# flyish/NoahGameFrame

Measured on AMD Instinct MI355X. Metric: entity-ticks/sec (update+dirty-diff+fanout) at 1M entities/GPU, 1/2/4/8 GPUs, higher is better.
Workload: dtype int64/f64; 1 GPU; BASELINE config[1]: 1048576 NPC/Player entities per GPU in one scene, 4096 groups x 256, 8 players/group, heartbeats HPRegen 1s/MPRegen 2s/Move 0.1s/Patrol 3s/Poison 0.5s, 100 ms frames; entities_per_gpu=1048576, groups=4096, players_per_group=8, parallelism=scene-shard x1

## Files before the change

### noahgameframe_amd/csrc/nfgpu_device.hpp

```cpp
#pragma once
#include <hip/hip_runtime.h>
#include <stdint.h>

#include "../../include/nfgpu.h"

namespace nfgpu {

constexpr int kTPB = 256;
constexpr int kTile = 256;
#ifndef NFGPU_RTILE
#define NFGPU_RTILE 64
#endif
constexpr int kRTile = NFGPU_RTILE;
static_assert(kRTile >= 1 && kRTile <= 64, "a record tile is at most one wave of slots");
constexpr uint32_t kRrcHost = 0x03FFFFFFu;
constexpr int kRrcSitShift = 26;

constexpr unsigned kErrMsgCap = 4, kErrTouch = 8, kErrFanBound = 16, kErrRemain = 32;

struct alignas(64) Ctrl {
    unsigned err, pad_u[3];
    unsigned long long n_ev, n_fi, n_re, n_msgs;
    unsigned long long msg_extent, n_msgs_ptiles;
    unsigned long long bytes_tick, bytes_rec, bytes_fan, pad2;
};

struct alignas(16) SchedHot {
    int64_t next;
    int32_t remain;
    uint32_t state;
};
constexpr uint32_t kStPresent = 1, kStForever = 2, kStFired = 4, kStStep = 8;
__host__ __device__ __forceinline__ int64_t st_step(uint32_t st) { return (int64_t)((int32_t)st >> 4); }
__host__ __device__ __forceinline__ uint32_t st_pack_step(int64_t step) {
    return (step >= -(1ll << 27) && step < (1ll << 27)) ? (kStStep | ((uint32_t)step << 4)) : 0u;
}
struct alignas(16) SchedCold {
    int64_t start;
    int32_t all;
    float interval;
};

constexpr unsigned kAblPrograms = 4;
constexpr unsigned kAblPerKind = 8;
constexpr unsigned kAblWaves6 = 16, kAblWaves8 = 32;
constexpr unsigned kAblWaves5 = 8192;
constexpr unsigned kAblNoRun = 512, kAblNoLoads = 1024, kAblNoEmit = 2048;
constexpr unsigned kAblNoWriteBack = 1u << 18, kAblNoSchedStore = 1u << 19;
constexpr unsigned kAblNoFiStore = 128, kAblNoEvStore = 256;
constexpr unsigned kAblGroupColumns = 1u << 20, kAblSigGroups = 1u << 21;
constexpr unsigned kAblNoPad = 1u << 22;
constexpr unsigned kAblFanWin16 = 1u << 24, kAblFanWin32 = 1u << 25;
constexpr unsigned kAblFan1 = 1u << 26;
constexpr unsigned kAblFanNoWin = 1u << 30;
constexpr unsigned kAblTinyTcap = 1u << 27;
constexpr unsigned kAblForceMsgCap = 1u << 29;
typedef uint32_t u32x4_a4 __attribute__((ext_vector_type(4), aligned(4)));
typedef uint32_t u32x2_a4 __attribute__((ext_vector_type(2), aligned(4)));
constexpr int64_t kColPad = 2304;
constexpr unsigned kAblScanInFrame = 131072;
constexpr unsigned kAblScanKernel = 1u << 28;
constexpr int kLbMaxTiles = 256;
constexpr unsigned kAblNoFuse = 4096;
constexpr unsigned kAblCheckRem = 64;
constexpr int32_t kRemUnset = (int32_t)0x80000001;

__host__ __device__ inline uint32_t rec_pos(uint64_t used, uint64_t rowm, int r) {
    const uint64_t below = (1ull << r) - 1;
    return ((used >> r) & 1) ? (uint32_t)__builtin_popcountll(used & below)
                             : (uint32_t)(__builtin_popcountll(used & rowm) + __builtin_popcountll(~used & rowm & below));
}
__host__ __device__ inline uint64_t rec_rowm(int rows) { return rows >= 64 ? ~0ull : ((1ull << rows) - 1); }

struct RecOp {
    int32_t kind, rec, col, code;
    int64_t a, b, c;
};

constexpr int kMaxU = 16, kMaxW = 12;
constexpr uint8_t kNoU = 0xFF;
constexpr int kCellPid = 0x10000;
constexpr uint32_t kNoCell = 0xFFFFFFFFu;
__host__ __device__ __forceinline__ uint32_t cell_rec(uint32_t c) { return (c >> 10) & 7u; }
__host__ __device__ __forceinline__ uint32_t cell_row(uint32_t c) { return (c >> 4) & 63u; }
__host__ __device__ __forceinline__ uint32_t cell_col(uint32_t c) { return c & 15u; }
// ... 110 lines not shown
    uint32_t ablate;
    RecOpX rops[NFK_MAX_REC_OPS];
    int32_t n_rops;
    uint32_t rop_kinds;
    unsigned long long* tally;
    int32_t n_w, n_u;
    int32_t u_pid[kMaxU];
    uint64_t* u_col[kMaxU];
    int32_t u_str[kMaxU];
    int32_t u_order[kMaxW];
    uint32_t u_lower[kMaxW];
    uint32_t u_cmask[NFK_MAX_CLASSES];
    int32_t n_tiles, n_rtiles;
    int32_t ev_tcap, fi_tcap, re_tcap;
    uint32_t* t_ev;
    uint32_t* t_fi;
    uint32_t* t_re;
    uint32_t* t_msg;
    uint32_t* ev_base;
    uint32_t* fi_base;
    uint32_t* re_base;
    uint32_t* msg_base;
    uint64_t* lb_st;
    uint32_t* lb_cnt;
    uint32_t lb_epoch;
    int32_t lb_rank;
    uint32_t msg_tcap;
    int32_t fuse_fan;
    int32_t fuse_rec;
    uint32_t msg_rb0, msg_rtcap;
    int32_t lds_words;
    int32_t xcd_map;
    uint32_t* ev_slot; uint32_t* ev_pid; uint64_t* ev_old; uint64_t* ev_new; uint32_t* ev_moff;
    uint32_t* fi_slot; uint32_t* fi_kind; int32_t* fi_remain;
    uint32_t* re_rrc; uint64_t* re_old; uint64_t* re_new; uint32_t* re_moff;
    uint32_t* msg_rcpt; int64_t msg_cap;
    uint64_t* ev_old_h; uint64_t* ev_new_h;
    unsigned* err_host;
};

constexpr int kErrHostWords = 16;
__device__ __forceinline__ void dev_error(const Dev& d, unsigned bit) {
    atomicOr(&d.ctrl->err, bit);
    if (d.err_host) __hip_atomic_store(d.err_host + __builtin_ctz(bit), 1u, __ATOMIC_RELAXED, __HIP_MEMORY_SCOPE_SYSTEM);
}

constexpr int kTallyN = 64, kTallyTick = 0, kTallyRec = 1, kTallyFan = 2;
// ... 120 lines not shown
```

### noahgameframe_amd/csrc/nfgpu_host.hip

```cpp
#include <algorithm>
#include <chrono>
#include <cmath>
#include <cstdlib>
#include <cstdio>
#include <cstring>
#include <functional>
#include <map>
#include <memory>
#include <numeric>
#include <string>
#include <unordered_map>
#include <vector>

#include <mutex>
#include <thread>

#include <rocprim/device/device_radix_sort.hpp>
#include <rocprim/device/device_scan.hpp>

#include "nfgpu_jit.hpp"
#include "nfgpu_kernels.hip"
#include "../../include/nfgpu_guidmap.hpp"
#include "nfgpu_pool.hpp"

// ... 959 lines not shown

std::mutex g_jit_mu;
std::map<std::string, std::pair<hipFunction_t, hipFunction_t>> g_jit;

void build_jit(World* w) {
    w->jit_fn = nullptr;
    w->jit_chain_fn = nullptr;
    const char* env = getenv("NFGPU_JIT");
    if (env && env[0] == '0') {
        w->jit_msg = "disabled (NFGPU_JIT=0)";
        return;
    }
    if (!w->u_ok) {
        w->jit_msg = "working set does not fit k_tick (k_tick_touch runs)";
        return;
    }
    const int u = std::max(w->d.n_u, 1);
    int waves = (w->d.ablate & (kAblWaves6 | kAblWaves8 | kAblWaves5)) ? tick_waves(w->d.n_u, w->d.ablate) : kWavesJit;
    if (const char* ew = getenv("NFGPU_JIT_WAVES")) waves = std::max(1, std::min(8, atoi(ew)));
    const char* es = getenv("NFGPU_JIT_SPEC");
    const bool spec = es && es[0] == '1';
    uint32_t nt = kJitNtDefault;
    if (const char* en = getenv("NFGPU_JIT_NT")) nt = (uint32_t)strtoul(en, nullptr, 0);
    bool lb = ((int64_t)std::max(w->d.N, 1) + kTile - 1) / kTile <= kLbMaxTiles;
    if (const char* el = getenv("NFGPU_JIT_LB")) lb = el[0] == '1';
    const std::string src = jit_schema_source(w->tab, w->d, spec, nt, lb);
    int dev = 0;
    (void)hipGetDevice(&dev);
    const std::string key = std::to_string(dev) + "|" + std::to_string(waves) + "|" + std::to_string(u) + "|" + src;
    std::lock_guard<std::mutex> lk(g_jit_mu);
    auto it = g_jit.find(key);
    if (it == g_jit.end()) {
        JitBuild b = jit_compile(src, waves, u);
        hipModule_t mod = nullptr;
        hipFunction_t fn = nullptr, cfn = nullptr;
        if (!b.ok || hipModuleLoadData(&mod, b.code.data()) != hipSuccess ||
            hipModuleGetFunction(&fn, mod, b.lowered.c_str()) != hipSuccess ||
            hipModuleGetFunction(&cfn, mod, b.lowered_chain.c_str()) != hipSuccess) {
            w->jit_msg = "hipRTC build failed: " + b.log.substr(0, 2000);
            return;
        }
        it = g_jit.emplace(key, std::make_pair(fn, cfn)).first;
    }
    w->jit_fn = it->second.first;
    w->jit_chain_fn = it->second.second;
    w->jit_lb = lb;
    w->jit_waves = waves;
// ... 988 lines not shown
    set_working_set(w);
    ALLOC(w->pl_slot_w, (size_t)cap * 4);
    ALLOC(w->slot_obj_d, (size_t)cap * 4);
    ALLOC(w->fan_desc_w, (size_t)cap * 8);
    d.fan_desc = w->fan_desc_w;
    {
        const char* ab = getenv("NFGPU_ABLATE");
        d.ablate = ab ? (uint32_t)strtoul(ab, nullptr, 0) : 0u;
    }
    d.pl_slot = w->pl_slot_w;
    d.ev_tcap = kTile * std::max(w->n_dst_union, 1);
    d.fi_tcap = kTile * std::max(NK, 1);
    d.re_tcap = (int32_t)(kRTile * std::max<size_t>(rec_events_per_ent, 1));
    const size_t nt = cap / kTile, nrt = cap / kRTile;
    const size_t ev_n = nt * d.ev_tcap, fi_n = nt * d.fi_tcap, re_n = d.has_recops ? nrt * d.re_tcap : 1;
    ALLOC(d.t_ev, nt * 4);
    ALLOC(d.t_fi, nt * 4);
    ALLOC(d.t_re, nrt * 4);
    ALLOC(d.t_msg, (nt + nrt) * 4);
    ALLOC(d.ev_base, (nt + 1) * 4);
    ALLOC(d.fi_base, (nt + 1) * 4);
    ALLOC(d.re_base, (nrt + 1) * 4);
    ALLOC(d.msg_base, (nt + nrt + 1) * 4);
    ALLOC(d.lb_st, std::min<size_t>(nt, kLbMaxTiles) * 4 * 8);
    ALLOC(d.lb_cnt, 64);
    d.msg_cap = w->cfg.msg_capacity > 0 ? w->cfg.msg_capacity : (int64_t)cap * 32;
    if (d.msg_cap > 0xFFFFFFFFll) return fail(NFK_ERR_ARG, "msg_capacity must fit 32-bit offsets");
    ALLOC(d.ev_slot, ev_n * 4);
    ALLOC(d.ev_pid, ev_n * 4);
    ALLOC(d.ev_old, ev_n * 8);
    ALLOC(d.ev_new, ev_n * 8);
    ALLOC(d.ev_moff, ev_n * 4);
    if (w->cfg.n_obj) {
        ALLOC(d.ev_old_h, ev_n * 8);
        ALLOC(d.ev_new_h, ev_n * 8);
    }
    ALLOC(d.fi_slot, fi_n * 4);
    ALLOC(d.fi_kind, fi_n * 4);
    ALLOC(d.fi_remain, fi_n * 4);
    ALLOC(d.re_rrc, re_n * 4);
    ALLOC(d.re_old, re_n * 8);
    ALLOC(d.re_new, re_n * 8);
    ALLOC(d.re_moff, re_n * 4);
    ALLOC(d.msg_rcpt, d.msg_cap * 4);
    d.tab = w->tab_d;
    d.ctrl = w->ctrl;
    d.n_rops = nro;
    d.rop_kinds = w->tab.kind_has_recop;
// ... 64 lines not shown
        std::vector<uint64_t> fd(cap, kDeadDesc);
        std::vector<int32_t> pls(cap, 0), so(cap, -1);
        for (size_t i = 0; i < meta.slot.size(); i++) {
            fd[meta.slot[i]] = meta.desc[i];
            pls[meta.slot[i]] = meta.pl[i];
            so[meta.slot[i]] = meta.obj[i];
        }
        HIPCHK(hipMemcpy(w->fan_desc_w, fd.data(), (size_t)cap * 8, hipMemcpyHostToDevice));
        HIPCHK(hipMemcpy(w->pl_slot_w, pls.data(), (size_t)cap * 4, hipMemcpyHostToDevice));
        HIPCHK(hipMemcpy(w->slot_obj_d, so.data(), (size_t)cap * 4, hipMemcpyHostToDevice));
    }
    HIPCHK(hipMemset(d.e_flags, 0, cap));
    HIPCHK(hipMemset(d.ext_head, 0, (size_t)cap * 4));
    HIPCHK(hipMemset(d.rs_head, 0, (size_t)cap * 4));
    HIPCHK(hipMemset(d.fired_mask, 0, (size_t)cap * 4));
    HIPCHK(hipMemset(d.t_ev, 0, nt * 4));
    HIPCHK(hipMemset(d.t_fi, 0, nt * 4));
    HIPCHK(hipMemset(d.t_re, 0, nrt * 4));
    HIPCHK(hipMemset(d.t_msg, 0, (nt + nrt) * 4));
    HIPCHK(hipMemset(d.ev_base, 0, (nt + 1) * 4));
    HIPCHK(hipMemset(d.fi_base, 0, (nt + 1) * 4));
    HIPCHK(hipMemset(d.re_base, 0, (nrt + 1) * 4));
    HIPCHK(hipMemset(d.msg_base, 0, (nt + nrt + 1) * 4));
    HIPCHK(hipMemset(d.lb_st, 0, std::min<size_t>(nt, kLbMaxTiles) * 4 * 8));
    HIPCHK(hipMemset(d.lb_cnt, 0, 64));
    w->lb_epoch = 0;
    for (auto& v : w->init_props) std::vector<uint64_t>().swap(v);
    for (auto& v : w->init_rcells) std::vector<uint64_t>().swap(v);
    build_jit(w);
    {
        const size_t room = (size_t)w->n_obj + (size_t)w->n_obj / 4 + 4096;
        w->gh.reserve(room);
        w->gd.reserve(room);
        w->guid.reserve(room);
        w->scene.reserve(room);
        w->group.reserve(room);
        w->cls.reserve(room);
        w->isplayer.reserve(room);
        w->slot_of_obj.reserve(room);
        w->alive.reserve(room);
        w->src_row.reserve(room);
        w->m_flag.reserve(room);
        if (!w->ins_rows) {
            const size_t c = 1024;
            HIPCHK(hipMalloc((void**)&w->ins_rows, c * (size_t)w->row_words * 8));
            w->ins_cap = c;
        }
    }
// ... 878 lines not shown
    return NFK_OK;
}

int nfk_import_objects(void* world, int32_t n, const int64_t* gh, const int64_t* gd, const int32_t* scene,
                       const int32_t* group, const uint8_t* cls, const uint8_t* isplayer, const uint64_t* rows_dev) {
    World* w = (World*)world;
    if (!w) return fail(NFK_ERR_ARG, "null world");
    return import_common(w, n, gh, gd, scene, group, cls, isplayer, rows_dev, hipMemcpyDeviceToDevice);
}

int nfk_spawn_objects(void* world, int32_t n, const int64_t* gh, const int64_t* gd, const int32_t* scene,
                      const int32_t* group, const uint8_t* cls, const uint8_t* isplayer, const uint64_t* props) {
    World* w = (World*)world;
    if (!w || (n > 0 && !props)) return fail(NFK_ERR_ARG, "null argument");
    if (!w->committed) return fail(NFK_ERR_STATE, "commit first (before it, use nfk_create_objects)");
    std::vector<uint64_t> rows((size_t)std::max(n, 0) * w->row_words, 0);
    for (int32_t i = 0; i < n; i++)
        memcpy(&rows[(size_t)i * w->row_words], props + (size_t)i * w->n_pw, (size_t)w->n_pw * 8);
    return import_common(w, n, gh, gd, scene, group, cls, isplayer, rows.data(), hipMemcpyHostToDevice);
}

static int execute_frame(World* w, int64_t now_ms, bool calls_only) {
    if (!w->committed) return fail(NFK_ERR_STATE, "commit first");
    if (const unsigned e = err_host_bits(w); e & (kErrFanBound | kErrTouch))
        return fail(NFK_ERR_DEVICE, std::string("device error of an earlier frame: ") +
                                        ((e & kErrFanBound) ? "a tile's fan-out exceeded its bound" : "touch list overflow") +
                                        " (nfk_summary_get reports and clears it)");
    using clk = std::chrono::steady_clock;
    const bool trace = getenv("NFGPU_TRACE_EXEC") != nullptr;
    clk::time_point tp[6];
    tp[0] = clk::now();
    {
        if (!w->mplan) w->mplan.reset(new MemPlan());
        MemPlan& mp = *w->mplan;
        int r = plan_membership(w, mp);
        if (r) return r;
        const int rf = check_fanout(w);
        r = commit_membership(w, mp);
        if (rf) return drop_window(w, rf);
        if (r) return drop_window(w, r);
    }
    if (const char* inj = getenv("NFGPU_INJECT_EXEC_FAIL"); inj && inj[0] == '1')
        return drop_window(w, fail(NFK_ERR_CAPACITY, "injected failure after the membership changes"));
    if (w->cfg.n_obj) w->xops_h.resize(w->xops.size(), 0);
    Dev d = w->d;
    d.now = now_ms;

    tp[1] = clk::now();
    const size_t n_xdev = w->xq_n, n_xq = n_xdev + w->xops.size(), n_hq = w->hops.size();
// ... 460 lines not shown
                                                       : w->last_rec_msgs + w->last_rec_msgs / 4) + 1024;
        if (tcap * d.n_tiles <= kMsgStrideLimit) {
            if (need > w->d.msg_cap) {
                HIPCHK(hipStreamSynchronize(w->stream));
                int r = regrow(w, (void**)&w->d.msg_rcpt, (size_t)need * 4);
                if (r) {
                    w->d.msg_cap = 0;
                    return drop_window(w, r);
                }
                w->d.msg_cap = need;
                d.msg_rcpt = w->d.msg_rcpt;
                d.msg_cap = need;
            }
            d.msg_tcap = (uint32_t)tcap;
            if (rfuse) {
                d.fuse_rec = 1;
                d.msg_rb0 = (uint32_t)(tcap * d.n_tiles);
                d.msg_rtcap = (uint32_t)rtcap;
            }
        }
    }
    d.fuse_fan = d.msg_tcap != 0;
    const bool cells = d.n_u > 0 && d.u_pid[d.n_u - 1] >= kCellPid;
    d.lb_rank = (d.fuse_fan && !d.has_recops && d.n_tiles && d.n_tiles <= kLbMaxTiles &&
                 !(d.ablate & kAblScanKernel) && (!(use_u && w->jit_fn) || w->jit_lb)) ? 1 : 0;
    if (d.lb_rank) {
        if (++w->lb_epoch == 0xFFFFFFFFu) {
            HIPCHK(hipMemsetAsync(w->d.lb_st, 0, std::min<size_t>(w->obj_of_slot.size() / kTile, kLbMaxTiles) * 4 * 8,
                                  w->stream));
            w->lb_epoch = 1;
        }
        d.lb_epoch = w->lb_epoch;
    }
    w->last_tcap = d.msg_tcap;
    w->last_rtcap = d.fuse_rec ? d.msg_rtcap : 0u;
    if (!calls_only) w->chain_ran = false;
    if (!calls_only && (w->chain_watch[0] | w->chain_watch[1]) && d.N) {
        uint32_t kinds = 0;
        int64_t wops = 0;
        for (int k = 0; k < d.n_kind; k++)
            for (int i = 0; i < w->tab.nops[k]; i++) {
                const nfk_op& op = w->tab.ops[k][i];
                const bool prop_op = op.code == NFK_OP_IADD_CLAMP || op.code == NFK_OP_FLERP ||
                                     op.code == NFK_OP_FAFFINE || op.code == NFK_OP_ISET || op.code == NFK_OP_FSET;
                if (prop_op && op.dst < 128 && ((w->chain_watch[op.dst >> 6] >> (op.dst & 63)) & 1)) {
                    kinds |= 1u << k;
                    wops++;
                }
            }
        static const bool no_closure = getenv("NFGPU_CHAIN_NO_CLOSURE") && getenv("NFGPU_CHAIN_NO_CLOSURE")[0] == '1';
        if (kinds && !no_closure) {
            auto bit = [](uint64_t (&m)[2], uint32_t p) {
// ... 78 lines not shown
                else hipLaunchKernelGGL((k_chain_u<16, DynSchema>), dim3((unsigned)nt), dim3(kTPB), 0, w->stream, d, cd, cc, tcap, kinds, w0, w1);
            } else {
                hipLaunchKernelGGL(k_chain, dim3((unsigned)nt), dim3(kTPB), 0, w->stream, d, w->chain_d, w->chain_cnt_d, tcap,
                                   kinds, w->chain_watch[0], w->chain_watch[1]);
            }
            HIPCHK(hipGetLastError());
            w->chain_ran = true;
            w->chain_tiles = nt;
        }
    }
    if (d.n_tiles) {
        TimeScope ts(w, KT_TICK);
        size_t lds = (size_t)std::max(d.n_w, 1) * kTPB * 8 + (size_t)std::max(d.n_kind, 1) * kTPB * 4;
        const bool jit = use_u && w->jit_fn;
        if (d.fuse_fan) {
            const int waves = jit ? w->jit_waves : tick_waves(d.n_u, d.ablate);
            lds = std::max(lds, (size_t)(163840 / waves - 2560) & ~(size_t)1023);
        }
        d.lds_words = (int32_t)(lds / 4);
        {
            static const int xm = getenv("NFGPU_TICK_XCD") ? atoi(getenv("NFGPU_TICK_XCD")) : 1;
            d.xcd_map = xm;
        }
        const dim3 g((unsigned)d.n_tiles), b(kTPB);
        if (jit) {
            void* args[] = {&d};
            HIPCHK(hipModuleLaunchKernel(w->jit_fn, (unsigned)d.n_tiles, 1, 1, kTPB, 1, 1, (unsigned)lds, w->stream,
                                         args, nullptr));
        } else if (use_u && cells) {
            if (d.n_u <= 8 && !(d.ablate & kAblWaves6))
                hipLaunchKernelGGL((k_tick<kWavesU8, 8, DynSchemaCells>), g, b, lds, w->stream, d);
            else if (d.n_u <= 12 && !(d.ablate & kAblWaves6))
                hipLaunchKernelGGL((k_tick<kWavesU12, 12, DynSchemaCells>), g, b, lds, w->stream, d);
            else
                hipLaunchKernelGGL((k_tick<6, 16, DynSchemaCells>), g, b, lds, w->stream, d);
        } else if (use_u && d.n_u <= 8 && !(d.ablate & kAblWaves6))
            hipLaunchKernelGGL((k_tick<kWavesU8, 8>), g, b, lds, w->stream, d);
        else if (use_u && d.n_u <= 12 && !(d.ablate & kAblWaves6))
            hipLaunchKernelGGL((k_tick<kWavesU12, 12>), g, b, lds, w->stream, d);
        else if (use_u)
            hipLaunchKernelGGL((k_tick<6, 16>), g, b, lds, w->stream, d);
        else
            hipLaunchKernelGGL(k_tick_touch, dim3((unsigned)d.n_tiles), dim3(kTPB), 0, w->stream, d);
        HIPCHK(hipGetLastError());
    }
    if (d.has_recops && d.n_rtiles) {
        TimeScope ts(w, KT_REC);
        constexpr int kWpb = kTPB / 64;
        const dim3 g((unsigned)((d.n_rtiles + kWpb - 1) / kWpb)), b(kTPB);
        if (nrss)
// ... 196 lines not shown
    }
    out->n_prop_events = (int64_t)c.n_ev;
    out->n_rec_events = (int64_t)c.n_re;
    out->n_fired = (int64_t)c.n_fi;
    out->n_msgs = frame_msgs(w, c);
    {
        out->alg_bytes_tick = (int64_t)(tb[0] - w->last_bytes[0]);
        out->alg_bytes_rec = (int64_t)(tb[1] - w->last_bytes[1]);
        out->alg_bytes_fan = (int64_t)(tb[2] - w->last_bytes[2]);
        for (int k = 0; k < 3; k++) w->last_bytes[k] = tb[k];
    }
    if ((c.err & kErrMsgCap) && !(c.err & ~kErrMsgCap)) {
        int r = regrow_fanout(w, c);
        if (r) return r;
    }
    w->last_rec_msgs = frame_msgs(w, c) - (int64_t)c.n_msgs_ptiles;
    out->device_error = (int32_t)c.err;
    out->tick = w->ticks;
    if (c.err) HIPCHK(hipMemset(&w->ctrl->err, 0, sizeof(unsigned)));
    clear_err_host(w);
    if (c.err & kErrTouch) return fail(NFK_ERR_TOUCH, "device touch list overflow");
    if (c.err & kErrFanBound) return fail(NFK_ERR_STATE, "a tile's fan-out exceeded its bound");
    if (c.err & kErrRemain) return fail(NFK_ERR_STATE, "k_tick read a fired heartbeat's remain it never wrote");
    if (c.err & kErrMsgCap)
        return fail(NFK_ERR_CAPACITY, "device output capacity exceeded (err=" + std::to_string(c.err) + ")");
    return NFK_OK;
}

int nfk_outputs_get(void* world, nfk_outputs* o) {
    World* w = (World*)world;
    if (!w || !o) return fail(NFK_ERR_ARG, "null argument");
    if (!w->committed) return fail(NFK_ERR_STATE, "commit first");
    int r = check_fanout(w);
    if (r) return r;
    if (const unsigned e = err_host_bits(w); e & (kErrFanBound | kErrTouch))
        return fail(NFK_ERR_DEVICE, (e & kErrFanBound) ? "a tile's fan-out exceeded its bound: the recipient lists are truncated"
                                                       : "touch list overflow: events are missing");
    r = ensure_ranks(w);
    if (r) return r;
    const Dev& d = w->d;
    o->n_tiles = d.n_tiles; o->tile_slots = kTile;
    o->n_rtiles = d.has_recops ? d.n_rtiles : 0; o->rtile_slots = kRTile;
    o->ev_tile_cap = d.ev_tcap; o->fi_tile_cap = d.fi_tcap; o->re_tile_cap = d.re_tcap;
    o->ev_base = d.ev_base; o->fi_base = d.fi_base; o->re_base = d.re_base; o->msg_base = d.msg_base;
    o->msg_cnt = d.t_msg;
    o->ev_slot = d.ev_slot; o->ev_pid = d.ev_pid; o->ev_old = d.ev_old; o->ev_new = d.ev_new;
    o->ev_moff = w->last_tcap ? nullptr : d.ev_moff;
    o->re_slot = nullptr;
    o->re_rrc = d.re_rrc; o->re_old = d.re_old; o->re_new = d.re_new;
    o->re_moff = w->last_rtcap ? nullptr : d.re_moff;
    o->fi_slot = d.fi_slot; o->fi_kind = d.fi_kind; o->fi_remain = d.fi_remain;
    o->msg_rcpt = d.msg_rcpt;
    o->slot_obj = w->slot_obj_d;
    o->ev_old_h = d.ev_old_h;
    o->ev_new_h = d.ev_new_h;
    return NFK_OK;
}

int nfk_read_object(void* world, int32_t pid, int64_t* head, int64_t* data) {
    World* w = (World*)world;
// ... 245 lines not shown
    for (int32_t i = 0; i < w->n_obj; i++) rank[w->guid_sorted[i]] = i;
    if ((size_t)w->n_obj > w->rank_cap) {
        HIPCHK(hipStreamSynchronize(w->stream));
        if (w->rank_d) HIPCHK(hipFree(w->rank_d));
        w->rank_d = nullptr;
        w->rank_cap = (size_t)w->n_obj + w->n_obj / 4 + 1024;
        HIPCHK(hipMalloc((void**)&w->rank_d, w->rank_cap * 4));
    }
    HIPCHK(hipMemcpy(w->rank_d, rank.data(), rank.size() * 4, hipMemcpyHostToDevice));
    w->rank_n = w->n_obj;
    return NFK_OK;
}

int nfk_read_frame(void* world, uint32_t what, nfk_frame_host* o) {
    World* w = (World*)world;
    if (!w || !o) return fail(NFK_ERR_ARG, "null argument");
    if (!w->committed) return fail(NFK_ERR_STATE, "commit first");
    memset(o, 0, sizeof *o);
    int r = check_fanout(w);
    if (r) return r;
    Ctrl c;
    r = read_ctrl(w, &c);
    if (r) return r;
    if (c.err & (kErrFanBound | kErrTouch))
        return fail(NFK_ERR_DEVICE, "the frame's outputs are incomplete (device error " + std::to_string(c.err) + ")");
    if (c.msg_extent > (unsigned long long)w->d.msg_cap) return fail(NFK_ERR_CAPACITY, "fan-out not recovered");
    const Dev& d = w->d;
    const bool fired = what & NFK_READ_FIRED, order = fired && (what & NFK_READ_FIRED_GUID_ORDER);
    const bool events = what & NFK_READ_EVENTS, fan = events && (what & NFK_READ_FANOUT);
    const bool heads = events && d.n_obj > 0;
    const size_t ne = events ? c.n_ev : 0, nr = events && d.has_recops ? c.n_re : 0, nf = fired ? c.n_fi : 0;
    const size_t nm = fan ? (size_t)frame_msgs(w, c) : 0;
    const int ntt = d.n_tiles + (d.has_recops ? d.n_rtiles : 0);
    size_t at = 0;
    auto take = [&](size_t bytes) {
        const size_t a = at;
        at += (bytes + 255) & ~(size_t)255;
        return a;
    };
    const size_t o_eo = take(ne * 4), o_ep = take(ne * 4), o_eold = take(ne * 8), o_enew = take(ne * 8);
    const size_t o_eoh = take(heads ? ne * 8 : 0), o_enh = take(heads ? ne * 8 : 0);
    const size_t o_ro = take(nr * 4), o_rr = take(nr * 4), o_rold = take(nr * 8), o_rnew = take(nr * 8);
    const size_t o_fo = take(nf * 4), o_fk = take(nf * 4), o_fr = take(nf * 4);
    const size_t o_mo = take(fan ? (ne + nr + 1) * 4 : 0), o_mr = take(nm * 4);
    const size_t total = at;
    const size_t s_db = 0, s_keys = (((size_t)ntt + 1) * 4 + 255) & ~(size_t)255;
    const size_t s_k2 = s_keys + ((nf * 8 + 255) & ~(size_t)255), s_i1 = s_k2 + ((nf * 8 + 255) & ~(size_t)255);
// ... 255 lines not shown
        tab->rec_cols[r] = rec_cols[r];
    }
    for (int k = 0; k < n_kind; k++)
        for (int i = 0; i < n_ops[k]; i++) {
            const nfk_op& op = tab->ops[k][i];
            if (!(op.flags & NFK_GUARD_CELL)) continue;
            const uint32_t c = op.guard & 0x1FFFu, r = cell_rec(c);
            if (!(op.flags & NFK_GUARD) || (op.guard & 0xE000u) || (int)r >= n_rec || (int)cell_row(c) >= rec_rows[r] ||
                (int)cell_col(c) >= rec_cols[r] || (col_types && col_types[(size_t)r * NFK_MAX_REC_COLS + cell_col(c)] != 0))
                return fail(NFK_ERR_ARG, "NFK_GUARD_CELL: not an int cell of a defined record");
        }
    std::vector<int> wp, rp;
    const bool u_ok = build_u_tables(*tab, n_kind, wp, rp);
    Dev d{};
    d.n_kind = n_kind;
    fill_u_dev(d, *tab, wp, rp, u_ok);
    if (!u_ok) {
        copy_msg("working set does not fit k_tick (k_tick_touch runs)", msg, msg_cap);
        return NFK_OK;
    }
    const char* es = getenv("NFGPU_JIT_SPEC");
    uint32_t nt = kJitNtDefault;
    if (const char* en = getenv("NFGPU_JIT_NT")) nt = (uint32_t)strtoul(en, nullptr, 0);
    const std::string s = jit_schema_source(*tab, d, es && es[0] == '1', nt);
    copy_msg(s, src, src_cap);
    if (!compile) {
        *ok = 1;
        return NFK_OK;
    }
    const int u = std::max(d.n_u, 1), waves = kWavesJit;
    JitBuild b = jit_compile(s, waves, u, true);
    *ok = b.ok;
    if (b.ok) {
        std::istringstream in(b.log);
        std::string line, other, usage_lines;
        const std::string tag = " [-Rpass-analysis=kernel-resource-usage]";
        bool in_remark = false;
        while (std::getline(in, line)) {
            const size_t r = line.find("remark: "), t = line.find(tag);
            if (r != std::string::npos && t != std::string::npos && t > r) {
                usage_lines += line.substr(r + 8, t - r - 8) + "\n";
                in_remark = true;
                continue;
            }
            if (line.find("warning:") != std::string::npos || line.find("error:") != std::string::npos) in_remark = false;
            if (!in_remark) other += line + "\n";
        }
// ... 66 lines not shown
```

### noahgameframe_amd/csrc/nfgpu_tick.hpp

```cpp
#pragma once
#include "nfgpu_device.hpp"

namespace nfgpu {

__device__ __forceinline__ int next_standalone(const Dev& d, int g, int e) {
    for (; g < d.n_x && d.x_slot[g] == (uint32_t)e; g++)
        if (d.tab->w_slot[d.x_pid[g]] == kNoU &&
            (d.x_old[g] != d.x_new[g] || ((int)d.x_pid[g] >= d.n_if && d.x_old_h[g] != d.x_new_h[g])))
            return g;
    return d.n_x;
}
struct EvFan {
    uint32_t n;
    bool pub;
};
__device__ __forceinline__ EvFan ev_fan(const Dev& d, uint64_t desc, uint32_t pid) {
    const uint8_t fl = d.tab->pflags[desc >> 60][pid];
    return EvFan{event_msgs(desc, fl), (fl & NFK_PUBLIC) != 0};
}

#define NFK_U16(X) X(0) X(1) X(2) X(3) X(4) X(5) X(6) X(7) X(8) X(9) X(10) X(11) X(12) X(13) X(14) X(15)
static_assert(kMaxU == 16, "NFK_U16 enumerates kMaxU slots");

__device__ __forceinline__ uint32_t uslot(uint32_t raw, uint32_t n_w) {
// ... 269 lines not shown
                        h[j].next = c.start + step * (int64_t)done;
                    }
                    h[j].state = st | kStFired;
                }
                if (s_rem) s_rem[k * kTPB + threadIdx.x] = h[j].remain;
                bytes += 16;
            }
        }
        if (kStore && fire && !(d.ablate & kAblNoSchedStore))
            st_nt<(S::kNt & kNtStateStore) != 0>(elem<S>(d.s_hot + (size_t)k * d.s_kstr, (uint32_t)e), h[j]);
    }
}
template <class S = DynSchema, bool kStore = true>
__device__ __forceinline__ uint32_t sched_scan(const Dev& d, int e, unsigned& bytes, uint64_t& desc,
                                               int32_t* s_rem = nullptr, bool oob = false) {
    uint32_t fired = 0;
    bool dead = true, taken = false;
    sched_chunk<S, true, kStore>(d, e, 0, bytes, desc, dead, taken, fired, s_rem, oob);
    for (int k0 = kKindChunk; k0 < S::n_kind(d); k0 += kKindChunk)
        sched_chunk<S, false, kStore>(d, e, k0, bytes, desc, dead, taken, fired, s_rem, oob);
    return fired;
}

__device__ __forceinline__ void lb_store(const Dev& d, int tile, int q, uint32_t v) {
    __hip_atomic_store(d.lb_st + (size_t)tile * 4 + q, ((uint64_t)d.lb_epoch << 32) | v, __ATOMIC_RELAXED,
                       __HIP_MEMORY_SCOPE_AGENT);
}
__device__ __forceinline__ uint32_t lb_load(const Dev& d, int tile, int q) {
    const uint64_t* p = d.lb_st + (size_t)tile * 4 + q;
    uint64_t s;
    while (((s = __hip_atomic_load(p, __ATOMIC_RELAXED, __HIP_MEMORY_SCOPE_AGENT)) >> 32) != d.lb_epoch)
        __builtin_amdgcn_s_sleep(1);
    return (uint32_t)s;
}
__device__ __forceinline__ bool lb_arrive(const Dev& d, int tile, uint32_t ev, uint32_t fi, uint32_t msg) {
    if (threadIdx.x < 3) lb_store(d, tile, threadIdx.x, threadIdx.x == 0 ? ev : threadIdx.x == 1 ? fi : msg);
    if (threadIdx.x != 0) return false;
    return __hip_atomic_fetch_add(d.lb_cnt, 1u, __ATOMIC_RELAXED, __HIP_MEMORY_SCOPE_AGENT) == (uint32_t)d.n_tiles - 1u;
}
__device__ void lb_scan_all(const Dev& d, unsigned long long* s_w) {
    static_assert(kLbMaxTiles <= kTPB, "one tile's counts per thread");
    const int n = d.n_tiles, t = (int)threadIdx.x;
    uint32_t ev = 0, fi = 0, ms = 0;
    if (t < n) {
        ev = lb_load(d, t, 0);
        fi = lb_load(d, t, 1);
        ms = lb_load(d, t, 2);
    }
    unsigned long long tef, tm;
    const unsigned long long xef = block_excl_scan(((unsigned long long)fi << 32) | ev, s_w, tef);
    __syncthreads();
    block_excl_scan(ms, s_w, tm);
    if (t < n) {
        d.ev_base[t] = (uint32_t)xef;
        d.fi_base[t] = (uint32_t)(xef >> 32);
        d.msg_base[t] = (uint32_t)t * d.msg_tcap;
    }
    if (t == 0) {
        const unsigned long long ext = (unsigned long long)n * d.msg_tcap;
        d.ev_base[n] = (uint32_t)tef;
        d.fi_base[n] = (uint32_t)(tef >> 32);
        d.msg_base[n] = (uint32_t)ext;
        d.re_base[0] = 0;
        d.ctrl->n_ev = (uint32_t)tef;
        d.ctrl->n_fi = (uint32_t)(tef >> 32);
        d.ctrl->n_re = 0;
        d.ctrl->msg_extent = ext;
        d.ctrl->n_msgs_ptiles = tm;
        if (ext > (unsigned long long)d.msg_cap || (d.ablate & kAblForceMsgCap)) dev_error(d, kErrMsgCap);
        __hip_atomic_store(d.lb_cnt, 0u, __ATOMIC_RELAXED, __HIP_MEMORY_SCOPE_AGENT);
    }
}

__device__ __forceinline__ int xcd_tile(int b, int n) {
    const int x = b & 7, i = b >> 3, q = n >> 3, r = n & 7;
    return x * q + min(x, r) + i;
}

template <int kU, class S>
__device__ __forceinline__ void tick_tile(const Dev& d, const int tile, unsigned long long* s_w, unsigned& s_bytes,
                                          uint32_t& s_lb_last, uint32_t* s_pb, uint64_t* s_o) {
    constexpr int kW = kU < kMaxW ? kU : kMaxW;
    const int e = tile * kTile + (int)threadIdx.x;
    if (d.tile_work && !d.tile_work[tile]) {
        if (d.has_recops && e < d.N) d.fired_mask[e] = 0;
        if (threadIdx.x == 0) {
            d.t_ev[tile] = 0;
            d.t_fi[tile] = 0;
            d.t_msg[tile] = 0;
        }
        if (S::kLb && d.lb_rank) {
            const bool last = lb_arrive(d, tile, 0u, 0u, 0u);
            if (threadIdx.x == 0) s_lb_last = last;
            __syncthreads();
            if (s_lb_last) lb_scan_all(d, s_w);
        }
        return;
    }
    const bool fuse = d.msg_tcap != 0;
    if (threadIdx.x == 0) {
        s_bytes = 0;
        s_pb[0] = 0xFFFFFFFFu;
        s_pb[1] = 0;
        s_pb[2] = 1;
    }
    int32_t* s_rem = (int32_t*)(s_o + (size_t)S::n_w(d) * kTPB);
    if (d.ablate & kAblCheckRem)
        for (int k = 0; k < S::n_kind(d); k++) s_rem[k * kTPB + threadIdx.x] = kRemUnset;
    unsigned bytes = 0;
    uint32_t fired = 0, xh = 0, wm = 0;
    uint64_t desc = kDeadDesc;
    uint64_t v[kU];
#pragma unroll
    for (int j = 0; j < kU; j++) v[j] = 0;
    {
        const int ec = e < d.N ? e : d.N - 1;
        if constexpr (S::kSpecMask != 0) {
            if (!(d.ablate & kAblNoLoads))
#pragma unroll
// ... 99 lines not shown
    const unsigned nf = __builtin_popcount(fired);
    const uint32_t dm_ = dm;
    unsigned long long tot;
    const unsigned long long excl =
        block_excl_scan(((unsigned long long)nf << 48) | ((unsigned long long)nd << 32) | nmsg, s_w, tot);
    const unsigned pev0 = (unsigned)((excl >> 32) & 0xFFFF);
    unsigned pfi = (unsigned)(excl >> 48);
    const unsigned pmsg0 = (unsigned)excl, tmsg = (unsigned)tot;
    if (fuse) {
        const uint32_t np = (uint32_t)((desc >> 32) & 0x3FFF);
        uint32_t lo = nmsg ? (uint32_t)desc : 0xFFFFFFFFu, hi = nmsg ? (uint32_t)desc + np : 0u;
#pragma unroll
        for (int m = 32; m >= 1; m >>= 1) {
            lo = min(lo, (uint32_t)__shfl_xor((int)lo, m, 64));
            hi = max(hi, (uint32_t)__shfl_xor((int)hi, m, 64));
            nmax = max(nmax, (uint32_t)__shfl_xor((int)nmax, m, 64));
        }
        if ((threadIdx.x & 63) == 0 && hi) {
            atomicMin(&s_pb[0], lo);
            atomicMax(&s_pb[1], hi);
            atomicMax(&s_pb[2], nmax);
        }
    }
    const bool lb_last = S::kLb && d.lb_rank && lb_arrive(d, tile, (unsigned)((tot >> 32) & 0xFFFF), (unsigned)(tot >> 48), tmsg);
    const size_t ev0 = (size_t)tile * d.ev_tcap, fi0 = (size_t)tile * d.fi_tcap;
    uint32_t* const t_evm = d.ev_moff + ev0;

    if (live) {
        if (nd && !(d.ablate & kAblNoEmit)) {
            uint32_t* const t_evs = d.ev_slot + ev0;
            uint32_t* const t_evp = d.ev_pid + ev0;
            uint64_t* const t_evo = d.ev_old + ev0;
            uint64_t* const t_evn = d.ev_new + ev0;
            if (!nsd) {
                constexpr bool kNE = (S::kNt & kNtEventStore) != 0;
                bool pend = false;
                uint32_t pa = 0, pp = 0;
                uint64_t po = 0, pn = 0;
#pragma unroll
                for (int j = 0; j < kW; j++) {
                    if (j >= S::n_w(d) || !((dm >> j) & 1)) continue;
                    const uint32_t below = dm & S::u_lower(d, j);
                    const uint32_t at = pev0 + __builtin_popcount(below);
                    const uint64_t nv = v[j], ov = s_o[j * kTPB + threadIdx.x];
                    const uint32_t pid = (uint32_t)S::u_pid(d, j);
                    if (!(d.ablate & kAblNoWriteBack)) st_nt<(S::kNt & kNtStateStore) != 0>(elem<S>(d.u_col[j], (uint32_t)e, S::u_str(d, j)), nv);
                    if (!fuse)
// ... 72 lines not shown
                dev_error(d, kErrRemain);
            if (!(d.ablate & kAblNoFiStore)) {
                st_off_nt<kNE>(t_fis, pfi, (uint32_t)e);
                st_off_nt<kNE>(t_fik, pfi, (uint32_t)k);
                st_off_nt<kNE>(t_fir, pfi, rem);
            }
            pfi++;
            bytes += 12;
        }
        if (xh) *elem<S>(d.ext_head, (uint32_t)e) = 0;
    }
    if (d.has_recops && e < d.N) {
        *elem<S>(d.fired_mask, (uint32_t)e) = fired;
        bytes += 4;
    }
    if (!fuse && !(d.ablate & kAblNoEmit)) bytes += 4 * nd;
    if (fuse) {
        __syncthreads();
        uint32_t dm = dm_;
        const unsigned mb = (unsigned)tile * d.msg_tcap;
        const unsigned tev = (unsigned)((tot >> 32) & 0xFFFF);
        const bool fan = tmsg && tmsg <= d.msg_tcap;
        if (tmsg > d.msg_tcap && threadIdx.x == 0) dev_error(d, kErrFanBound);
        if (fan) {
            const unsigned R = (unsigned)d.lds_words;
            const uint32_t pb_lo = s_pb[0], npl = s_pb[1] > s_pb[0] ? s_pb[1] - s_pb[0] : 0u;
            const uint32_t nm = s_pb[2];
            const uint32_t L = nm <= 1 ? 1u : nm >= 64 ? 64u : 1u << (32 - __builtin_clz(nm - 1));
            const uint32_t sub = threadIdx.x & (L - 1);
            const bool win = !(d.ablate & kAblFanNoWin) &&
                             L < ((d.ablate & kAblFanWin32) ? 64u : (d.ablate & kAblFanWin16) ? 32u : 16u);
            const bool staged = npl <= R / 4;
            const unsigned room = R - (staged ? npl : 0u);
            const unsigned ecap = (min(tev, win ? room / 6u : room / 3u) + 3u) & ~3u;
            const unsigned W = win ? (room - 3u * ecap) & ~3u : 0u;
            uint32_t* s_ev = (uint32_t*)s_o;
            uint32_t* s_win = s_ev + 3u * ecap;
            uint32_t* s_pl = s_ev + (R - npl);
            uint32_t* out = d.msg_rcpt + mb;
            if (staged) {
                for (uint32_t i = threadIdx.x; i < npl; i += kTPB) s_pl[i] = (uint32_t)d.pl_slot[pb_lo + i];
                bytes += 4 * ((npl + kTPB - 1 - threadIdx.x) / kTPB);
            }
            bytes += 4 * nmsg;
            for (unsigned c0 = 0; c0 < tev; c0 += ecap) {
                const unsigned c1 = min(tev, c0 + ecap);
// ... 90 lines not shown
                                k++;
                            }
                        }
                        __syncthreads();
                        const uint32_t n = w1 - w0;
                        if ((w0 & 3u) == 0) {
                            const uint32_t n4 = n >> 2;
                            uint4* dst4 = (uint4*)(out + w0);
                            const uint4* src4 = (const uint4*)s_win;
                            for (uint32_t i = threadIdx.x; i < n4; i += kTPB) st_nt<(S::kNt & kNtFanStore) != 0>(dst4 + i, src4[i]);
                            if (threadIdx.x < (n & 3u)) out[w0 + 4 * n4 + threadIdx.x] = s_win[4 * n4 + threadIdx.x];
                        } else {
                            for (uint32_t i = threadIdx.x; i < n; i += kTPB) out[w0 + i] = s_win[i];
                        }
                        __syncthreads();
                    }
                }
                if (c1 < tev) __syncthreads();
            }
        }
    }
    const unsigned wb = (unsigned)wave_sum(bytes);
    if ((threadIdx.x & 63) == 0) atomicAdd(&s_bytes, wb);
    if (S::kLb && threadIdx.x == 0) s_lb_last = lb_last;
    __syncthreads();
    const bool lb_scan = S::kLb && d.lb_rank && s_lb_last;
    if (threadIdx.x == 0) {
        d.t_ev[tile] = (unsigned)((tot >> 32) & 0xFFFF);
        d.t_fi[tile] = (unsigned)(tot >> 48);
        d.t_msg[tile] = (unsigned)tot;
        tally_add(d, kTallyTick, (unsigned long long)(s_bytes + 12 + (fuse ? 16 : 0)));
    }
    if constexpr (S::kLb)
        if (lb_scan) lb_scan_all(d, s_w);
}

template <int kWPE, int kU, class S = DynSchema>
__global__ __launch_bounds__(kTPB) __attribute__((amdgpu_waves_per_eu(kWPE, 8))) void k_tick(Dev d) {
    __shared__ unsigned long long s_w[kTPB / 64];
    __shared__ unsigned s_bytes;
    __shared__ uint32_t s_lb_last;
    __shared__ uint32_t s_pb[3];
    extern __shared__ __align__(16) uint64_t s_o[];
    const int tile = d.xcd_map ? xcd_tile((int)blockIdx.x, d.n_tiles) : (int)blockIdx.x;
    tick_tile<kU, S>(d, tile, s_w, s_bytes, s_lb_last, s_pb, s_o);
}


struct ChainEnt {
    uint32_t slot;
    uint16_t pid;
    uint8_t kind, op;
    uint64_t old_bits, new_bits;
};
static_assert(sizeof(ChainEnt) == 24, "ChainEnt is read back as 24-byte records");

template <int kU, class S>
__global__ __launch_bounds__(kTPB) void k_chain_u(Dev d, ChainEnt* __restrict__ out, uint32_t* __restrict__ t_cnt,
                                                  uint32_t tcap, uint32_t kinds, uint64_t watch0, uint64_t watch1) {
    __shared__ unsigned long long s_w[kTPB / 64];
    const int e = blockIdx.x * kTPB + (int)threadIdx.x;
    uint32_t fired = 0;
    uint64_t v[kU];
#pragma unroll
    for (int j = 0; j < kU; j++) v[j] = 0;
    if (e < d.N) {
        unsigned bytes = 0;
        uint64_t desc = kDeadDesc;
// ... 39 lines not shown
```

Measured before the change: 13.26 billion entity-ticks/s.

## Replace last-tile-arrives scan with dedicated rank workgroups polling per-tile counts

The in-kernel tile-count scan (load-balanced ranking) was limited to 256 tiles and ran in the last-arriving tile. It is replaced by two extra workgroups appended to the k_tick grid. Each one polls the per-tile published counts with a timeout and computes the exclusive scans, one for ev/fi and one for msg. At 1M entities (4096 tiles) this enables in-kernel ranking where a separate scan kernel used to run, removing a launch and a round trip. The cost is that the rank workgroups spin while tiles finish, which relies on forward progress. A timeout error path is added in case they give up waiting.

```diff
diff --git a/noahgameframe_amd/csrc/nfgpu_device.hpp b/noahgameframe_amd/csrc/nfgpu_device.hpp
--- a/noahgameframe_amd/csrc/nfgpu_device.hpp
+++ b/noahgameframe_amd/csrc/nfgpu_device.hpp
@@ -16,7 +16,7 @@
 constexpr uint32_t kRrcHost = 0x03FFFFFFu;
 constexpr int kRrcSitShift = 26;
 
-constexpr unsigned kErrMsgCap = 4, kErrTouch = 8, kErrFanBound = 16, kErrRemain = 32;
+constexpr unsigned kErrMsgCap = 4, kErrTouch = 8, kErrFanBound = 16, kErrRemain = 32, kErrRankWait = 64;
 
 struct alignas(64) Ctrl {
     unsigned err, pad_u[3];
@@ -60,7 +60,7 @@
 constexpr int64_t kColPad = 2304;
 constexpr unsigned kAblScanInFrame = 131072;
 constexpr unsigned kAblScanKernel = 1u << 28;
-constexpr int kLbMaxTiles = 256;
+constexpr unsigned kAblRankPer1 = 1u << 23;
 constexpr unsigned kAblNoFuse = 4096;
 constexpr unsigned kAblCheckRem = 64;
 constexpr int32_t kRemUnset = (int32_t)0x80000001;
@@ -217,7 +217,6 @@
     uint32_t* re_base;
     uint32_t* msg_base;
     uint64_t* lb_st;
-    uint32_t* lb_cnt;
     uint32_t lb_epoch;
     int32_t lb_rank;
     uint32_t msg_tcap;
diff --git a/noahgameframe_amd/csrc/nfgpu_host.hip b/noahgameframe_amd/csrc/nfgpu_host.hip
--- a/noahgameframe_amd/csrc/nfgpu_host.hip
+++ b/noahgameframe_amd/csrc/nfgpu_host.hip
@@ -1005,7 +1005,7 @@
     const bool spec = es && es[0] == '1';
     uint32_t nt = kJitNtDefault;
     if (const char* en = getenv("NFGPU_JIT_NT")) nt = (uint32_t)strtoul(en, nullptr, 0);
-    bool lb = ((int64_t)std::max(w->d.N, 1) + kTile - 1) / kTile <= kLbMaxTiles;
+    bool lb = !w->d.has_recops && !(w->d.ablate & kAblScanKernel);
     if (const char* el = getenv("NFGPU_JIT_LB")) lb = el[0] == '1';
     const std::string src = jit_schema_source(w->tab, w->d, spec, nt, lb);
     int dev = 0;
@@ -2040,8 +2040,7 @@
     ALLOC(d.fi_base, (nt + 1) * 4);
     ALLOC(d.re_base, (nrt + 1) * 4);
     ALLOC(d.msg_base, (nt + nrt + 1) * 4);
-    ALLOC(d.lb_st, std::min<size_t>(nt, kLbMaxTiles) * 4 * 8);
-    ALLOC(d.lb_cnt, 64);
+    ALLOC(d.lb_st, std::max<size_t>(nt, 1) * kRankWgs * 8);
     d.msg_cap = w->cfg.msg_capacity > 0 ? w->cfg.msg_capacity : (int64_t)cap * 32;
     if (d.msg_cap > 0xFFFFFFFFll) return fail(NFK_ERR_ARG, "msg_capacity must fit 32-bit offsets");
     ALLOC(d.ev_slot, ev_n * 4);
@@ -2152,8 +2151,7 @@
     HIPCHK(hipMemset(d.fi_base, 0, (nt + 1) * 4));
     HIPCHK(hipMemset(d.re_base, 0, (nrt + 1) * 4));
     HIPCHK(hipMemset(d.msg_base, 0, (nt + nrt + 1) * 4));
-    HIPCHK(hipMemset(d.lb_st, 0, std::min<size_t>(nt, kLbMaxTiles) * 4 * 8));
-    HIPCHK(hipMemset(d.lb_cnt, 0, 64));
+    HIPCHK(hipMemset(d.lb_st, 0, std::max<size_t>(nt, 1) * kRankWgs * 8));
     w->lb_epoch = 0;
     for (auto& v : w->init_props) std::vector<uint64_t>().swap(v);
     for (auto& v : w->init_rcells) std::vector<uint64_t>().swap(v);
@@ -3078,9 +3076,11 @@
 
 static int execute_frame(World* w, int64_t now_ms, bool calls_only) {
     if (!w->committed) return fail(NFK_ERR_STATE, "commit first");
-    if (const unsigned e = err_host_bits(w); e & (kErrFanBound | kErrTouch))
+    if (const unsigned e = err_host_bits(w); e & (kErrFanBound | kErrTouch | kErrRankWait))
         return fail(NFK_ERR_DEVICE, std::string("device error of an earlier frame: ") +
-                                        ((e & kErrFanBound) ? "a tile's fan-out exceeded its bound" : "touch list overflow") +
+                                        ((e & kErrFanBound) ? "a tile's fan-out exceeded its bound"
+                                         : (e & kErrTouch)  ? "touch list overflow"
+                                                            : "k_tick's rank workgroups gave up waiting") +
                                         " (nfk_summary_get reports and clears it)");
     using clk = std::chrono::steady_clock;
     const bool trace = getenv("NFGPU_TRACE_EXEC") != nullptr;
@@ -3587,12 +3587,13 @@
     }
     d.fuse_fan = d.msg_tcap != 0;
     const bool cells = d.n_u > 0 && d.u_pid[d.n_u - 1] >= kCellPid;
-    d.lb_rank = (d.fuse_fan && !d.has_recops && d.n_tiles && d.n_tiles <= kLbMaxTiles &&
-                 !(d.ablate & kAblScanKernel) && (!(use_u && w->jit_fn) || w->jit_lb)) ? 1 : 0;
+    if (d.fuse_fan && !d.has_recops && d.n_tiles && !(d.ablate & kAblScanKernel) && (!(use_u && w->jit_fn) || w->jit_lb))
+        d.lb_rank = (d.n_tiles <= kTPB || (d.ablate & kAblRankPer1)) ? 1 : kRankPer;
+    else
+        d.lb_rank = 0;
     if (d.lb_rank) {
         if (++w->lb_epoch == 0xFFFFFFFFu) {
-            HIPCHK(hipMemsetAsync(w->d.lb_st, 0, std::min<size_t>(w->obj_of_slot.size() / kTile, kLbMaxTiles) * 4 * 8,
-                                  w->stream));
+            HIPCHK(hipMemsetAsync(w->d.lb_st, 0, std::max<size_t>((size_t)d.cap / kTile, 1) * kRankWgs * 8, w->stream));
             w->lb_epoch = 1;
         }
         d.lb_epoch = w->lb_epoch;
@@ -3717,10 +3718,10 @@
             static const int xm = getenv("NFGPU_TICK_XCD") ? atoi(getenv("NFGPU_TICK_XCD")) : 1;
             d.xcd_map = xm;
         }
-        const dim3 g((unsigned)d.n_tiles), b(kTPB);
+        const dim3 g((unsigned)(d.n_tiles + (d.lb_rank ? kRankWgs : 0))), b(kTPB);
         if (jit) {
             void* args[] = {&d};
-            HIPCHK(hipModuleLaunchKernel(w->jit_fn, (unsigned)d.n_tiles, 1, 1, kTPB, 1, 1, (unsigned)lds, w->stream,
+            HIPCHK(hipModuleLaunchKernel(w->jit_fn, g.x, 1, 1, kTPB, 1, 1, (unsigned)lds, w->stream,
                                          args, nullptr));
         } else if (use_u && cells) {
             if (d.n_u <= 8 && !(d.ablate & kAblWaves6))
@@ -3963,6 +3964,7 @@
     if (c.err & kErrTouch) return fail(NFK_ERR_TOUCH, "device touch list overflow");
     if (c.err & kErrFanBound) return fail(NFK_ERR_STATE, "a tile's fan-out exceeded its bound");
     if (c.err & kErrRemain) return fail(NFK_ERR_STATE, "k_tick read a fired heartbeat's remain it never wrote");
+    if (c.err & kErrRankWait) return fail(NFK_ERR_DEVICE, "k_tick's rank workgroups gave up waiting for a tile's counts: the frame has no ranks");
     if (c.err & kErrMsgCap)
         return fail(NFK_ERR_CAPACITY, "device output capacity exceeded (err=" + std::to_string(c.err) + ")");
     return NFK_OK;
@@ -3974,9 +3976,10 @@
     if (!w->committed) return fail(NFK_ERR_STATE, "commit first");
     int r = check_fanout(w);
     if (r) return r;
-    if (const unsigned e = err_host_bits(w); e & (kErrFanBound | kErrTouch))
+    if (const unsigned e = err_host_bits(w); e & (kErrFanBound | kErrTouch | kErrRankWait))
         return fail(NFK_ERR_DEVICE, (e & kErrFanBound) ? "a tile's fan-out exceeded its bound: the recipient lists are truncated"
-                                                       : "touch list overflow: events are missing");
+                                    : (e & kErrTouch)  ? "touch list overflow: events are missing"
+                                                       : "k_tick's rank workgroups gave up waiting: the frame has no ranks");
     r = ensure_ranks(w);
     if (r) return r;
     const Dev& d = w->d;
@@ -4268,7 +4271,7 @@
     Ctrl c;
     r = read_ctrl(w, &c);
     if (r) return r;
-    if (c.err & (kErrFanBound | kErrTouch))
+    if (c.err & (kErrFanBound | kErrTouch | kErrRankWait))
         return fail(NFK_ERR_DEVICE, "the frame's outputs are incomplete (device error " + std::to_string(c.err) + ")");
     if (c.msg_extent > (unsigned long long)w->d.msg_cap) return fail(NFK_ERR_CAPACITY, "fan-out not recovered");
     const Dev& d = w->d;
@@ -4570,7 +4573,9 @@
     const char* es = getenv("NFGPU_JIT_SPEC");
     uint32_t nt = kJitNtDefault;
     if (const char* en = getenv("NFGPU_JIT_NT")) nt = (uint32_t)strtoul(en, nullptr, 0);
-    const std::string s = jit_schema_source(*tab, d, es && es[0] == '1', nt);
+    bool lb = true;
+    if (const char* el = getenv("NFGPU_JIT_LB")) lb = el[0] == '1';
+    const std::string s = jit_schema_source(*tab, d, es && es[0] == '1', nt, lb);
     copy_msg(s, src, src_cap);
     if (!compile) {
         *ok = 1;
diff --git a/noahgameframe_amd/csrc/nfgpu_tick.hpp b/noahgameframe_amd/csrc/nfgpu_tick.hpp
--- a/noahgameframe_amd/csrc/nfgpu_tick.hpp
+++ b/noahgameframe_amd/csrc/nfgpu_tick.hpp
@@ -315,53 +315,94 @@
     return fired;
 }
 
+constexpr int kRankWgs = 2;
+constexpr int kRankPer = 16;
+constexpr unsigned long long kRankWaitTicks = 100000000ull;
+
 __device__ __forceinline__ void lb_store(const Dev& d, int tile, int q, uint32_t v) {
-    __hip_atomic_store(d.lb_st + (size_t)tile * 4 + q, ((uint64_t)d.lb_epoch << 32) | v, __ATOMIC_RELAXED,
-                       __HIP_MEMORY_SCOPE_AGENT);
-}
-__device__ __forceinline__ uint32_t lb_load(const Dev& d, int tile, int q) {
-    const uint64_t* p = d.lb_st + (size_t)tile * 4 + q;
-    uint64_t s;
-    while (((s = __hip_atomic_load(p, __ATOMIC_RELAXED, __HIP_MEMORY_SCOPE_AGENT)) >> 32) != d.lb_epoch)
-        __builtin_amdgcn_s_sleep(1);
-    return (uint32_t)s;
-}
-__device__ __forceinline__ bool lb_arrive(const Dev& d, int tile, uint32_t ev, uint32_t fi, uint32_t msg) {
-    if (threadIdx.x < 3) lb_store(d, tile, threadIdx.x, threadIdx.x == 0 ? ev : threadIdx.x == 1 ? fi : msg);
-    if (threadIdx.x != 0) return false;
-    return __hip_atomic_fetch_add(d.lb_cnt, 1u, __ATOMIC_RELAXED, __HIP_MEMORY_SCOPE_AGENT) == (uint32_t)d.n_tiles - 1u;
-}
-__device__ void lb_scan_all(const Dev& d, unsigned long long* s_w) {
-    static_assert(kLbMaxTiles <= kTPB, "one tile's counts per thread");
+    __hip_atomic_store(d.lb_st + (size_t)q * (size_t)(d.cap / kTile) + tile, ((uint64_t)d.lb_epoch << 32) | v,
+                       __ATOMIC_RELAXED, __HIP_MEMORY_SCOPE_AGENT);
+}
+__device__ __forceinline__ void lb_publish(const Dev& d, int tile, uint32_t ev, uint32_t fi, uint32_t msg) {
+    if (threadIdx.x < 2) lb_store(d, tile, threadIdx.x, threadIdx.x == 0 ? (fi << 16) | ev : msg);
+}
+template <int kPer>
+__device__ void lb_rank_wg(const Dev& d, const int q, unsigned long long* s_w, unsigned& s_late) {
     const int n = d.n_tiles, t = (int)threadIdx.x;
-    uint32_t ev = 0, fi = 0, ms = 0;
-    if (t < n) {
-        ev = lb_load(d, t, 0);
-        fi = lb_load(d, t, 1);
-        ms = lb_load(d, t, 2);
-    }
-    unsigned long long tef, tm;
-    const unsigned long long xef = block_excl_scan(((unsigned long long)fi << 32) | ev, s_w, tef);
+    if (t == 0) s_late = 0;
     __syncthreads();
-    block_excl_scan(ms, s_w, tm);
-    if (t < n) {
-        d.ev_base[t] = (uint32_t)xef;
-        d.fi_base[t] = (uint32_t)(xef >> 32);
-        d.msg_base[t] = (uint32_t)t * d.msg_tcap;
+    const uint64_t* const p = d.lb_st + (size_t)q * (size_t)(d.cap / kTile);
+    unsigned long long carry = 0;
+    for (int c0 = 0; c0 < n; c0 += kTPB * kPer) {
+        const int i0 = c0 + t * kPer;
+        uint64_t x[kPer];
+        uint32_t stale = 0;
+#pragma unroll
+        for (int j = 0; j < kPer; j++) {
+            x[j] = (uint64_t)d.lb_epoch << 32;
+            if (i0 + j < n) stale |= 1u << j;
+        }
+        bool late = false;
+        const unsigned long long t0 = __builtin_amdgcn_s_memrealtime();
+        while (stale) {
+#pragma unroll
+            for (int j = 0; j < kPer; j++)
+                if ((stale >> j) & 1u) x[j] = __hip_atomic_load(p + i0 + j, __ATOMIC_RELAXED, __HIP_MEMORY_SCOPE_AGENT);
+#pragma unroll
+            for (int j = 0; j < kPer; j++)
+                if ((uint32_t)(x[j] >> 32) == d.lb_epoch) stale &= ~(1u << j);
+            if (!stale) break;
+            if (__builtin_amdgcn_s_memrealtime() - t0 > kRankWaitTicks) {
+                late = true;
+                break;
+            }
+            __builtin_amdgcn_s_sleep(8);
+        }
+        if (late) s_late = 1;
+        __syncthreads();
+        if (s_late) {
+            if (late) dev_error(d, kErrRankWait);
+            return;
+        }
+        unsigned long long sum = 0;
+#pragma unroll
+        for (int j = 0; j < kPer; j++) {
+            const uint32_t v = (uint32_t)x[j];
+            x[j] = q == 0 ? ((unsigned long long)(v >> 16) << 32) | (v & 0xFFFFu) : v;
+            sum += x[j];
+        }
+        unsigned long long tot;
+        unsigned long long run = carry + block_excl_scan(sum, s_w, tot);
+#pragma unroll
+        for (int j = 0; j < kPer; j++) {
+            if (i0 + j < n) {
+                if (q == 0) {
+                    d.ev_base[i0 + j] = (uint32_t)run;
+                    d.fi_base[i0 + j] = (uint32_t)(run >> 32);
+                } else {
+                    d.msg_base[i0 + j] = (uint32_t)(i0 + j) * d.msg_tcap;
+                }
+            }
+            run += x[j];
+        }
+        carry += tot;
+        __syncthreads();
     }
     if (t == 0) {
-        const unsigned long long ext = (unsigned long long)n * d.msg_tcap;
-        d.ev_base[n] = (uint32_t)tef;
-        d.fi_base[n] = (uint32_t)(tef >> 32);
-        d.msg_base[n] = (uint32_t)ext;
-        d.re_base[0] = 0;
-        d.ctrl->n_ev = (uint32_t)tef;
-        d.ctrl->n_fi = (uint32_t)(tef >> 32);
-        d.ctrl->n_re = 0;
-        d.ctrl->msg_extent = ext;
-        d.ctrl->n_msgs_ptiles = tm;
-        if (ext > (unsigned long long)d.msg_cap || (d.ablate & kAblForceMsgCap)) dev_error(d, kErrMsgCap);
-        __hip_atomic_store(d.lb_cnt, 0u, __ATOMIC_RELAXED, __HIP_MEMORY_SCOPE_AGENT);
+        if (q == 0) {
+            d.ev_base[n] = (uint32_t)carry;
+            d.fi_base[n] = (uint32_t)(carry >> 32);
+            d.re_base[0] = 0;
+            d.ctrl->n_ev = (uint32_t)carry;
+            d.ctrl->n_fi = (uint32_t)(carry >> 32);
+            d.ctrl->n_re = 0;
+        } else {
+            const unsigned long long ext = (unsigned long long)n * d.msg_tcap;
+            d.msg_base[n] = (uint32_t)ext;
+            d.ctrl->msg_extent = ext;
+            d.ctrl->n_msgs_ptiles = carry;
+            if (ext > (unsigned long long)d.msg_cap || (d.ablate & kAblForceMsgCap)) dev_error(d, kErrMsgCap);
+        }
     }
 }
 
@@ -372,7 +413,7 @@
 
 template <int kU, class S>
 __device__ __forceinline__ void tick_tile(const Dev& d, const int tile, unsigned long long* s_w, unsigned& s_bytes,
-                                          uint32_t& s_lb_last, uint32_t* s_pb, uint64_t* s_o) {
+                                          uint32_t* s_pb, uint64_t* s_o) {
     constexpr int kW = kU < kMaxW ? kU : kMaxW;
     const int e = tile * kTile + (int)threadIdx.x;
     if (d.tile_work && !d.tile_work[tile]) {
@@ -382,12 +423,7 @@
             d.t_fi[tile] = 0;
             d.t_msg[tile] = 0;
         }
-        if (S::kLb && d.lb_rank) {
-            const bool last = lb_arrive(d, tile, 0u, 0u, 0u);
-            if (threadIdx.x == 0) s_lb_last = last;
-            __syncthreads();
-            if (s_lb_last) lb_scan_all(d, s_w);
-        }
+        if (S::kLb && d.lb_rank) lb_publish(d, tile, 0u, 0u, 0u);
         return;
     }
     const bool fuse = d.msg_tcap != 0;
@@ -533,7 +569,6 @@
             atomicMax(&s_pb[2], nmax);
         }
     }
-    const bool lb_last = S::kLb && d.lb_rank && lb_arrive(d, tile, (unsigned)((tot >> 32) & 0xFFFF), (unsigned)(tot >> 48), tmsg);
     const size_t ev0 = (size_t)tile * d.ev_tcap, fi0 = (size_t)tile * d.fi_tcap;
     uint32_t* const t_evm = d.ev_moff + ev0;
 
@@ -652,6 +687,7 @@
         const unsigned tev = (unsigned)((tot >> 32) & 0xFFFF);
         const bool fan = tmsg && tmsg <= d.msg_tcap;
         if (tmsg > d.msg_tcap && threadIdx.x == 0) dev_error(d, kErrFanBound);
+        if (S::kLb && d.lb_rank) lb_publish(d, tile, tev, (unsigned)(tot >> 48), tmsg);
         if (fan) {
             const unsigned R = (unsigned)d.lds_words;
             const uint32_t pb_lo = s_pb[0], npl = s_pb[1] > s_pb[0] ? s_pb[1] - s_pb[0] : 0u;
@@ -788,28 +824,31 @@
     }
     const unsigned wb = (unsigned)wave_sum(bytes);
     if ((threadIdx.x & 63) == 0) atomicAdd(&s_bytes, wb);
-    if (S::kLb && threadIdx.x == 0) s_lb_last = lb_last;
     __syncthreads();
-    const bool lb_scan = S::kLb && d.lb_rank && s_lb_last;
     if (threadIdx.x == 0) {
         d.t_ev[tile] = (unsigned)((tot >> 32) & 0xFFFF);
         d.t_fi[tile] = (unsigned)(tot >> 48);
         d.t_msg[tile] = (unsigned)tot;
         tally_add(d, kTallyTick, (unsigned long long)(s_bytes + 12 + (fuse ? 16 : 0)));
     }
-    if constexpr (S::kLb)
-        if (lb_scan) lb_scan_all(d, s_w);
 }
 
 template <int kWPE, int kU, class S = DynSchema>
 __global__ __launch_bounds__(kTPB) __attribute__((amdgpu_waves_per_eu(kWPE, 8))) void k_tick(Dev d) {
     __shared__ unsigned long long s_w[kTPB / 64];
     __shared__ unsigned s_bytes;
-    __shared__ uint32_t s_lb_last;
     __shared__ uint32_t s_pb[3];
     extern __shared__ __align__(16) uint64_t s_o[];
+    if constexpr (S::kLb) {
+        if ((int)blockIdx.x >= d.n_tiles) {
+            const int q = (int)blockIdx.x - d.n_tiles;
+            if (d.lb_rank == 1) lb_rank_wg<1>(d, q, s_w, s_bytes);
+            else lb_rank_wg<kRankPer>(d, q, s_w, s_bytes);
+            return;
+        }
+    }
     const int tile = d.xcd_map ? xcd_tile((int)blockIdx.x, d.n_tiles) : (int)blockIdx.x;
-    tick_tile<kU, S>(d, tile, s_w, s_bytes, s_lb_last, s_pb, s_o);
+    tick_tile<kU, S>(d, tile, s_w, s_bytes, s_pb, s_o);
 }
 
 
```

Result: faster. 14.09 billion entity-ticks/s, median of 6 (+6.2%).
